# chenxy99/Scanpaths

Hardware: AMD Instinct MI355X
Metric: images/sec/GPU (AiR train step, bs=32, 320x512) at 1/2/4/8 MI355X (higher is better)
Workload: dtype f32; 1 GPU; AiR supervised train step (fwd+loss+bwd+clip+Adam), resnet50, T=16, 320x512, per-GPU batch 32; global_batch=32, parallelism=dp1

## Files before the change

scanpaths_amd/csrc/bn_pool.hip:

```cpp
#include "common.h"
#include <algorithm>

namespace {

__device__ __forceinline__ int64_t sp_cdiv_dev(int64_t a, int64_t b) { return (a + b - 1) / b; }

constexpr int CB = 64;
constexpr int RL = 16;
constexpr int MAX_G = 256;

inline int pick_G_wide(int64_t M, int C) {
    const int64_t colblocks = sp_cdiv(C, 256);
    int64_t g = sp_cdiv(1024, colblocks);
    g = std::min<int64_t>(g, sp_cdiv(M, 4 * 8));
    g = std::min<int64_t>(g, 1024);
    return (int)std::max<int64_t>(g, 1);
}

inline int pick_G(int64_t M, int C) {
    const int64_t colblocks = sp_cdiv(C, CB);
    int64_t g = sp_cdiv(2048, colblocks);
    g = std::min<int64_t>(g, sp_cdiv(M, RL * 8));
    g = std::min<int64_t>(g, MAX_G);
    return (int)std::max<int64_t>(g, 1);
// ... 631 lines not shown
__global__ __launch_bounds__(256) void maxpool_fwd_kernel(const float* x, int N, int H, int W, int C, float* y, int Ho,
                                                          int Wo, unsigned char* amx) {
    const int C4 = C / 4;
    const int64_t total = (int64_t)N * Ho * Wo * C4;
    for (int64_t i = (int64_t)blockIdx.x * blockDim.x + threadIdx.x; i < total; i += (int64_t)gridDim.x * blockDim.x) {
        const int c4 = (int)(i % C4);
        int64_t r = i / C4;
        const int xo = (int)(r % Wo); r /= Wo;
        const int yo = (int)(r % Ho);
        const int n = (int)(r / Ho);
        float4 m = make_float4(-INFINITY, -INFINITY, -INFINITY, -INFINITY);
        uchar4 am = make_uchar4(0, 0, 0, 0);
        for (int ky = 0; ky < 3; ++ky) {
            const int iy = yo * 2 + ky;
            if (iy >= H) break;
            for (int kx = 0; kx < 3; ++kx) {
                const int ix = xo * 2 + kx;
                if (ix >= W) break;
                const float4 a = *reinterpret_cast<const float4*>(x + (((int64_t)n * H + iy) * W + ix) * C + c4 * 4);
                const unsigned char q = (unsigned char)(ky * 3 + kx);
                if (a.x > m.x) { m.x = a.x; am.x = q; }
                if (a.y > m.y) { m.y = a.y; am.y = q; }
                if (a.z > m.z) { m.z = a.z; am.z = q; }
                if (a.w > m.w) { m.w = a.w; am.w = q; }
            }
        }
        reinterpret_cast<float4*>(y)[i] = m;
        if (amx) reinterpret_cast<uchar4*>(amx)[i] = am;
    }
}

__global__ __launch_bounds__(256) void maxpool_bwd_idx_kernel(const float* dy, const unsigned char* amx, int N, int H, int W,
                                                              int C, float* dx, int Ho, int Wo) {
    const int C4 = C / 4;
    const int64_t total = (int64_t)N * H * W * C4;
    for (int64_t i = (int64_t)blockIdx.x * blockDim.x + threadIdx.x; i < total; i += (int64_t)gridDim.x * blockDim.x) {
        const int c4 = (int)(i % C4);
        int64_t r = i / C4;
        const int ix = (int)(r % W); r /= W;
        const int iy = (int)(r % H);
        const int n = (int)(r / H);
        float4 g = make_float4(0.f, 0.f, 0.f, 0.f);
        const int oy_lo = max(0, (iy - 1) / 2), oy_hi = min(Ho - 1, iy / 2);
        const int ox_lo = max(0, (ix - 1) / 2), ox_hi = min(Wo - 1, ix / 2);
        for (int oy = oy_lo; oy <= oy_hi; ++oy) {
            if (iy - 2 * oy > 2) continue;
            for (int ox = ox_lo; ox <= ox_hi; ++ox) {
                if (ix - 2 * ox > 2) continue;
                const int64_t o = (((int64_t)n * Ho + oy) * Wo + ox) * C4 + c4;
                const uchar4 a = reinterpret_cast<const uchar4*>(amx)[o];
                const unsigned char mine = (unsigned char)((iy - 2 * oy) * 3 + (ix - 2 * ox));
                if (a.x == mine || a.y == mine || a.z == mine || a.w == mine) {
                    const float4 d = reinterpret_cast<const float4*>(dy)[o];
                    g.x += a.x == mine ? d.x : 0.f;
                    g.y += a.y == mine ? d.y : 0.f;
                    g.z += a.z == mine ? d.z : 0.f;
                    g.w += a.w == mine ? d.w : 0.f;
                }
            }
        }
        reinterpret_cast<float4*>(dx)[i] = g;
    }
}

__global__ __launch_bounds__(256) void nchw_to_nhwc_pad_kernel(const float* x, int N, int C, int H, int W, int Cp, float* y) {
    const int64_t total = (int64_t)N * H * W * Cp;
    for (int64_t i = (int64_t)blockIdx.x * blockDim.x + threadIdx.x; i < total; i += (int64_t)gridDim.x * blockDim.x) {
        const int c = (int)(i % Cp);
        int64_t r = i / Cp;
        const int w = (int)(r % W); r /= W;
        const int hh = (int)(r % H);
        const int n = (int)(r / H);
        y[i] = c < C ? x[(((int64_t)n * C + c) * H + hh) * W + w] : 0.f;
    }
}
__global__ __launch_bounds__(256) void pad_lastdim_kernel(const float* x, int64_t rows, int Cin, int Cout, float* y) {
    const int64_t total = rows * Cout;
    for (int64_t i = (int64_t)blockIdx.x * blockDim.x + threadIdx.x; i < total; i += (int64_t)gridDim.x * blockDim.x) {
        const int c = (int)(i % Cout);
        const int64_t r = i / Cout;
        y[i] = c < Cin ? x[r * Cin + c] : 0.f;
    }
}
__global__ __launch_bounds__(256) void add_kernel(const float* a, const float* b, float* o, int64_t n4) {
    for (int64_t i = (int64_t)blockIdx.x * blockDim.x + threadIdx.x; i < n4; i += (int64_t)gridDim.x * blockDim.x) {
        const float4 u = reinterpret_cast<const float4*>(a)[i], v = reinterpret_cast<const float4*>(b)[i];
        reinterpret_cast<float4*>(o)[i] = make_float4(u.x + v.x, u.y + v.y, u.z + v.z, u.w + v.w);
    }
}
struct SumList {
    const float* p[32];
    int n;
    const int* row_last;
    int step[32];
// ... 262 lines not shown
extern "C" int sp_rowsum(const float* x, int64_t M, int C, float scale, float* out, void* stream) {
    if (!x || !out) return SP_ENULL;
    if (C % 4) return SP_EINVAL;
    const int blocks = (int)std::max<int64_t>(1, std::min<int64_t>(sp_cdiv(M, 4), 4096));
    hipLaunchKernelGGL(rowsum_kernel, dim3(blocks), dim3(256), 0, (hipStream_t)stream, x, M, C, scale, out);
    SP_LAUNCH_CHECK();
    return SP_OK;
}

extern "C" int sp_rowsum_bwd(const float* dout, int64_t M, int C, float scale, float* dx, void* stream) {
    if (!dout || !dx) return SP_ENULL;
    if (C % 4) return SP_EINVAL;
    const int64_t n4 = M * C / 4;
    hipLaunchKernelGGL(rowsum_bwd_kernel, dim3(ew_blocks(n4)), dim3(256), 0, (hipStream_t)stream, dout, n4, C, scale, dx);
    SP_LAUNCH_CHECK();
    return SP_OK;
}

extern "C" int sp_maxpool3s2_fwd(const float* x, int N, int H, int W, int C, float* y, unsigned char* argmax, int Ho, int Wo,
                                 void* stream) {
    if (!x || !y) return SP_ENULL;
    if (C % 4) return SP_EINVAL;
    const int64_t total = (int64_t)N * Ho * Wo * (C / 4);
    hipLaunchKernelGGL(maxpool_fwd_kernel, dim3(ew_blocks(total)), dim3(256), 0, (hipStream_t)stream, x, N, H, W, C, y, Ho, Wo,
                       argmax);
    SP_LAUNCH_CHECK();
    return SP_OK;
}

extern "C" int sp_maxpool3s2_bwd(const float* dy, const unsigned char* argmax, int N, int H, int W, int C, float* dx, int Ho,
                                 int Wo, void* stream) {
    if (!dy || !argmax || !dx) return SP_ENULL;
    if (C % 4) return SP_EINVAL;
    const int64_t total = (int64_t)N * H * W * (C / 4);
    hipLaunchKernelGGL(maxpool_bwd_idx_kernel, dim3(ew_blocks(total) * 4), dim3(256), 0, (hipStream_t)stream, dy, argmax, N, H, W,
                       C, dx, Ho, Wo);
    SP_LAUNCH_CHECK();
    return SP_OK;
}

extern "C" int sp_nchw_to_nhwc_pad(const float* x, int N, int C, int H, int W, int Cp, float* y, void* stream) {
    if (!x || !y) return SP_ENULL;
    if (Cp < C) return SP_EINVAL;
    const int64_t total = (int64_t)N * H * W * Cp;
    hipLaunchKernelGGL(nchw_to_nhwc_pad_kernel, dim3(ew_blocks(total)), dim3(256), 0, (hipStream_t)stream, x, N, C, H, W, Cp, y);
    SP_LAUNCH_CHECK();
    return SP_OK;
}

extern "C" int sp_pad_lastdim(const float* x, int64_t rows, int Cin, int Cout, float* y, void* stream) {
    if (!x || !y) return SP_ENULL;
    const int64_t total = rows * Cout;
    hipLaunchKernelGGL(pad_lastdim_kernel, dim3(ew_blocks(total)), dim3(256), 0, (hipStream_t)stream, x, rows, Cin, Cout, y);
    SP_LAUNCH_CHECK();
    return SP_OK;
}

extern "C" int sp_add(const float* a, const float* b, float* out, int64_t n, void* stream) {
    if (!a || !b || !out) return SP_ENULL;
    const int64_t n4 = n / 4;
    if (n4 > 0) {
        hipLaunchKernelGGL(add_kernel, dim3(ew_blocks(n4)), dim3(256), 0, (hipStream_t)stream, a, b, out, n4);
        SP_LAUNCH_CHECK();
    }
    if (n4 * 4 < n) {
        hipLaunchKernelGGL(add_tail_kernel, dim3(1), dim3(256), 0, (hipStream_t)stream, a, b, out, n4 * 4, n);
        SP_LAUNCH_CHECK();
// ... 57 lines not shown
```

scanpaths_amd/csrc/decoder.hip:

```cpp
#include "common.h"
#include <algorithm>

namespace {

inline int ew_blocks(int64_t n) { return (int)std::max<int64_t>(1, std::min<int64_t>(sp_cdiv(n, 256), 2048)); }

__device__ __forceinline__ float sigmoidf_(float x) { return sp_sigmoid(x); }

__global__ __launch_bounds__(256) void lstm_fwd_kernel(const float* xg, const float* hg, const float* c_prev,
                                                       int64_t rows, int C, float* gates, float* c_out, float* h_out) {
    const int C4 = C / 4;
    const int64_t total = rows * C4;
    for (int64_t idx = (int64_t)blockIdx.x * blockDim.x + threadIdx.x; idx < total; idx += (int64_t)gridDim.x * blockDim.x) {
        const int64_t r = idx / C4;
        const int c = (int)(idx - r * C4) * 4;
        const float* px = xg + r * 4 * C + c;
        float4 pi = *reinterpret_cast<const float4*>(px);
        float4 pf = *reinterpret_cast<const float4*>(px + C);
        float4 po = *reinterpret_cast<const float4*>(px + 2 * C);
        float4 pg = *reinterpret_cast<const float4*>(px + 3 * C);
        if (hg) {
            const float* ph = hg + r * 4 * C + c;
            const float4 a = *reinterpret_cast<const float4*>(ph), b = *reinterpret_cast<const float4*>(ph + C);
            const float4 d = *reinterpret_cast<const float4*>(ph + 2 * C), e = *reinterpret_cast<const float4*>(ph + 3 * C);
            pi.x += a.x; pi.y += a.y; pi.z += a.z; pi.w += a.w;
            pf.x += b.x; pf.y += b.y; pf.z += b.z; pf.w += b.w;
            po.x += d.x; po.y += d.y; po.z += d.z; po.w += d.w;
            pg.x += e.x; pg.y += e.y; pg.z += e.z; pg.w += e.w;
        }
        float4 cp = make_float4(0.f, 0.f, 0.f, 0.f);
        if (c_prev) cp = *reinterpret_cast<const float4*>(c_prev + r * C + c);
        float4 gi, gf, go, gg, cn, hn;
#define CELL(k)                                   \
        gi.k = sigmoidf_(pi.k);                   \
        gf.k = sigmoidf_(pf.k);                   \
        go.k = sigmoidf_(po.k);                   \
        gg.k = sp_tanh(pg.k);                       \
        cn.k = gf.k * cp.k + gi.k * gg.k;         \
        hn.k = go.k * cn.k;
        CELL(x) CELL(y) CELL(z) CELL(w)
#undef CELL
        float* pgt = gates + r * 4 * C + c;
        *reinterpret_cast<float4*>(pgt) = gi;
        *reinterpret_cast<float4*>(pgt + C) = gf;
        *reinterpret_cast<float4*>(pgt + 2 * C) = go;
        *reinterpret_cast<float4*>(pgt + 3 * C) = gg;
        *reinterpret_cast<float4*>(c_out + r * C + c) = cn;
        *reinterpret_cast<float4*>(h_out + r * C + c) = hn;
    }
}

constexpr int SP_PCH = 160;
__global__ __launch_bounds__(256) void sempool_fwd_kernel(const float* __restrict__ a, const float* __restrict__ vf, int S, int B,
                                                          int P, int C, float* __restrict__ partial) {
    __shared__ f32x4 red[2][128];
    const int ch = blockIdx.x, b = blockIdx.y, nch = gridDim.x;
    const int c4 = threadIdx.x & 127, pl = threadIdx.x >> 7, C4 = C / 4;
    const int p0 = ch * SP_PCH, p1 = min(P, p0 + SP_PCH);
    f32x4 acc0 = {0.f, 0.f, 0.f, 0.f}, acc1 = {0.f, 0.f, 0.f, 0.f};
    if (c4 < C4)
        for (int p = p0 + pl; p < p1; p += 2) {
            const f32x4 v = *reinterpret_cast<const f32x4*>(vf + ((int64_t)b * P + p) * C + c4 * 4);
            acc0 += a[((int64_t)0 * B + b) * P + p] * v;
            if (S > 1) acc1 += a[((int64_t)1 * B + b) * P + p] * v;
        }
    if (pl == 1) { red[0][c4] = acc0; red[1][c4] = acc1; }
    __syncthreads();
    if (pl == 0 && c4 < C4) {
        acc0 += red[0][c4];
        acc1 += red[1][c4];
        f32x4* dst = reinterpret_cast<f32x4*>(partial + (((int64_t)ch * B + b) * S) * C) + c4;
        dst[0] = acc0;
        if (S > 1) dst[C4] = acc1;
    }
    (void)nch;
}
__global__ __launch_bounds__(256) void sempool_finish_kernel(const float* __restrict__ partial, int nch, int64_t n, float alpha,
                                                             float* __restrict__ out, int S, int C, int64_t osb, int64_t oss) {
    for (int64_t i = (int64_t)blockIdx.x * 256 + threadIdx.x; i < n; i += (int64_t)gridDim.x * 256) {
        float s = 0.f;
        for (int k = 0; k < nch; ++k) s += partial[(int64_t)k * n + i];
        const int c = (int)(i % C);
        const int64_t bs = i / C;
        out[(bs / S) * osb + (bs % S) * oss + c] = fmaxf(alpha * s, 0.f);
    }
}
__global__ __launch_bounds__(256) void sempool_bwd_kernel(const float* __restrict__ dz, const float* __restrict__ out,
                                                          const float* __restrict__ a, const float* __restrict__ vf, int S,
                                                          int B, int P, int C, float alpha, float* __restrict__ da,
                                                          float* __restrict__ dvf, const int* __restrict__ row_last, int row_step,
                                                          int64_t zsb, int64_t zss) {
    const int lane = threadIdx.x & 63;
    const int64_t wave = ((int64_t)blockIdx.x * 256 + threadIdx.x) >> 6, nwaves = ((int64_t)gridDim.x * 256) >> 6;
    const int nq = C / 4;
    for (int64_t bp = wave; bp < (int64_t)B * P; bp += nwaves) {
        const int b = (int)(bp / P), p = (int)(bp % P);
        if (row_last && row_last[b] < row_step) {
            for (int q = lane; q < nq; q += 64) *reinterpret_cast<f32x4*>(dvf + bp * C + q * 4) = f32x4{0.f, 0.f, 0.f, 0.f};
// ... 279 lines not shown
        const int x = (int)(q % W); q /= W;
        const int y = (int)(q % H);
        const int r = (int)(q / H);
        float v = 0.f;
        if (k < 9 * S) {
            const int s = k / 9, tap = k - 9 * s;
            const int yy = y + tap / 3 - 1, xx = x + tap % 3 - 1;
            if ((unsigned)yy < (unsigned)H && (unsigned)xx < (unsigned)W) v = maps[(((int64_t)s * R + r) * H + yy) * W + xx];
        }
        col[i] = v;
    }
}
__global__ __launch_bounds__(256) void col2im1_multi_kernel(const float* __restrict__ dcol, int S, int R, int H, int W, int ldk, float* __restrict__ dmaps) {
    const int64_t total = (int64_t)S * R * H * W;
    for (int64_t i = (int64_t)blockIdx.x * blockDim.x + threadIdx.x; i < total; i += (int64_t)gridDim.x * blockDim.x) {
        int64_t q = i;
        const int x = (int)(q % W); q /= W;
        const int y = (int)(q % H); q /= H;
        const int r = (int)(q % R);
        const int s = (int)(q / R);
        float acc = 0.f;
#pragma unroll
        for (int tap = 0; tap < 9; ++tap) {
            const int y0 = y - (tap / 3 - 1), x0 = x - (tap % 3 - 1);
            if ((unsigned)y0 < (unsigned)H && (unsigned)x0 < (unsigned)W)
                acc += dcol[(((int64_t)r * H + y0) * W + x0) * ldk + 9 * s + tap];
        }
        dmaps[i] = acc;
    }
}

constexpr int MAXT = 40;

__global__ __launch_bounds__(256) void listatt_fwd_kernel(const float* L, const float* u, int T, int R, int D, float* mem,
                                                          float* alpha) {
    __shared__ float sh16[16];
    __shared__ float sc[MAXT];
    const int r = blockIdx.x;
    for (int t0 = 0; t0 < T; t0 += 4) {
        float s[4] = {0.f, 0.f, 0.f, 0.f};
        for (int d = threadIdx.x; d < D; d += 256) {
            const float ud = u[d];
#pragma unroll
            for (int k = 0; k < 4; ++k)
                if (t0 + k < T) s[k] += L[((int64_t)(t0 + k) * R + r) * D + d] * ud;
        }
        block_sum4_256(s, sh16);
        if (threadIdx.x == 0) {
#pragma unroll
            for (int k = 0; k < 4; ++k)
                if (t0 + k < T) sc[t0 + k] = s[k];
        }
    }
    __syncthreads();
    float mx = -INFINITY;
    for (int t = 0; t < T; ++t) mx = fmaxf(mx, sc[t]);
    float den = 0.f;
    for (int t = 0; t < T; ++t) den += expf(sc[t] - mx);
    const float inv = 1.f / den;
    if (threadIdx.x < T) alpha[(int64_t)threadIdx.x * R + r] = expf(sc[threadIdx.x] - mx) * inv;
    for (int d = threadIdx.x; d < D; d += 256) {
        float acc = 0.f;
        for (int t = 0; t < T; ++t) acc += expf(sc[t] - mx) * inv * L[((int64_t)t * R + r) * D + d];
        mem[(int64_t)r * D + d] = acc;
    }
}

__global__ __launch_bounds__(256) void listatt_bwd_kernel(const float* dmem, const float* L, const float* u,
                                                          const float* alpha, int T, int R, int D, float* dL,
                                                          float* du_partial) {
    __shared__ float sh16[16];
    __shared__ float gs[MAXT];
    const int r = blockIdx.x;
    const float* dm = dmem + (int64_t)r * D;
    for (int t0 = 0; t0 < T; t0 += 4) {
        float s[4] = {0.f, 0.f, 0.f, 0.f};
        for (int d = threadIdx.x; d < D; d += 256) {
            const float dmd = dm[d];
#pragma unroll
            for (int k = 0; k < 4; ++k)
                if (t0 + k < T) s[k] += L[((int64_t)(t0 + k) * R + r) * D + d] * dmd;
        }
        block_sum4_256(s, sh16);
        if (threadIdx.x == 0) {
#pragma unroll
            for (int k = 0; k < 4; ++k)
                if (t0 + k < T) gs[t0 + k] = s[k];
        }
    }
    __syncthreads();
    float mean = 0.f;
    for (int t = 0; t < T; ++t) mean += alpha[(int64_t)t * R + r] * gs[t];
    for (int d = threadIdx.x; d < D; d += 256) {
        const float dmd = dm[d], ud = u[d];
        float du = 0.f;
        for (int t = 0; t < T; ++t) {
// ... 310 lines not shown
                                     const unsigned* dc_amax, float c_bound, float cprev_bound, void* planes,
                                     float* dpre_scale, const int* row_last, int row_step, int rows_per_sample, void* stream) {
    if (!gates || !c_out || (!dpre && !planes) || !dc_prev) return SP_ENULL;
    if (C % 4) return SP_EINVAL;
    if (planes && (!dpre_scale || C % 256 || ((uintptr_t)planes & 15) || (dh && !dh_amax) || (dc && !dc_amax))) return SP_EINVAL;
    if (row_last && (rows_per_sample < 1 || rows % rows_per_sample)) return SP_EINVAL;
    SP_RESET_AMAX(dpre_amax, stream);
    SP_RESET_AMAX(dcp_amax, stream);
    hipLaunchKernelGGL(lstm_bwd_kernel, dim3(ew_blocks(rows * C / 4)), dim3(256), 0, (hipStream_t)stream, dh, dc, gates,
                       c_prev, c_out, rows, C, dpre, dc_prev, dpre_amax, dcp_amax, dh_amax, dc_amax, c_bound, cprev_bound,
                       (uint16_t*)planes, dpre_scale, row_last, row_step, row_last ? rows_per_sample : 1);
    SP_LAUNCH_CHECK();
    return SP_OK;
}

extern "C" int sp_im2col3x3_1ch(const float* maps, int S, int R, int H, int W, int ldk, float* col, void* stream) {
    if (!maps || !col) return SP_ENULL;
    if (S < 1 || 9 * S > ldk) return SP_EINVAL;
    hipLaunchKernelGGL(im2col1_multi_kernel, dim3(ew_blocks((int64_t)R * H * W * ldk)), dim3(256), 0, (hipStream_t)stream, maps, S, R, H, W, ldk, col);
    SP_LAUNCH_CHECK();
    return SP_OK;
}
extern "C" int sp_col2im3x3_1ch(const float* dcol, int S, int R, int H, int W, int ldk, float* dmaps, void* stream) {
    if (!dcol || !dmaps) return SP_ENULL;
    if (S < 1 || 9 * S > ldk) return SP_EINVAL;
    hipLaunchKernelGGL(col2im1_multi_kernel, dim3(ew_blocks((int64_t)S * R * H * W)), dim3(256), 0, (hipStream_t)stream, dcol, S, R, H, W, ldk, dmaps);
    SP_LAUNCH_CHECK();
    return SP_OK;
}

extern "C" int sp_listatt_fwd(const float* L, const float* u, int T, int R, int D, float* mem, float* alpha, void* stream) {
    if (!L || !u || !mem || !alpha) return SP_ENULL;
    if (T < 1 || T > MAXT) return SP_EINVAL;
    hipLaunchKernelGGL(listatt_fwd_kernel, dim3(R), dim3(256), 0, (hipStream_t)stream, L, u, T, R, D, mem, alpha);
    SP_LAUNCH_CHECK();
    return SP_OK;
}

extern "C" int sp_listatt_bwd(const float* dmem, const float* L, const float* u, const float* alpha, int T, int R, int D,
                              float* dL, float* du_partial, void* stream) {
    if (!dmem || !L || !u || !alpha || !dL || !du_partial) return SP_ENULL;
    if (T < 1 || T > MAXT) return SP_EINVAL;
    hipLaunchKernelGGL(listatt_bwd_kernel, dim3(R), dim3(256), 0, (hipStream_t)stream, dmem, L, u, alpha, T, R, D, dL,
                       du_partial);
    SP_LAUNCH_CHECK();
    return SP_OK;
}

extern "C" int sp_mulrelu_fwd(const float* a, const float* b, int64_t n, int64_t nb, float* out, void* stream) {
    if (!a || !b || !out) return SP_ENULL;
    hipLaunchKernelGGL(mulrelu_fwd_kernel, dim3(ew_blocks(n)), dim3(256), 0, (hipStream_t)stream, a, b, n, nb, out);
    SP_LAUNCH_CHECK();
    return SP_OK;
}

extern "C" int sp_mulrelu_bwd(const float* dout, const float* a, const float* b, const float* out, int64_t n, int64_t nb,
                              float* da, float* db_partial, void* stream) {
    if (!dout || !a || !b || !out || !da || !db_partial) return SP_ENULL;
    hipLaunchKernelGGL(mulrelu_bwd_kernel, dim3(ew_blocks(n)), dim3(256), 0, (hipStream_t)stream, dout, a, b, out, n, nb, da,
                       db_partial);
    SP_LAUNCH_CHECK();
    return SP_OK;
}

extern "C" int sp_select_rows(const float* a, const float* b, const unsigned char* sel, int64_t rows, int64_t len, float* out,
                              void* stream) {
    if (!a || !b || !sel || !out) return SP_ENULL;
// ... 57 lines not shown
```

scanpaths_amd/csrc/head_direct.hip:

```cpp
#include "common.h"

namespace {

constexpr int NTAP = 49, NV = 121, MAXSITE = 32, MAXCLS = 8;

struct AxisCls {
    int n;
    int ncls;
    int len;
    unsigned char mask[MAXCLS];
    unsigned char cls[MAXSITE];
};

static bool make_axis(int len, AxisCls& a) {
    a.n = sp_drt_sites(len);
    a.ncls = 0;
    a.len = len;
    if (a.n < 1 || a.n > MAXSITE) return false;
    for (int s = 0; s < a.n; ++s) {
        unsigned m = 0;
        for (int k = 0; k < 7; ++k) {
            const int pos = 5 * s - 2 + k;
            if (pos >= 0 && pos < len) m |= 1u << k;
        }
// ... 36 lines not shown
        float s = 0.f;
        for (int ky = 0; ky < 7; ++ky)
            for (int kx = 0; kx < 7; ++kx)
                if (((my >> ky) & 1u) && ((mx >> kx) & 1u)) s += cb[(int64_t)hd * HC + 2 + ky * 7 + kx];
        cbsum[hd * ncls + cls] = s;
    }
}

__global__ __launch_bounds__(128) void compose11_bwd_kernel(const float* __restrict__ dW11, const float* __restrict__ dcbsum,
                                                            int HC, int C4, int ncls, AxisCls ay, AxisCls ax,
                                                            float* __restrict__ dG, float* __restrict__ dcb) {
    const int u = blockIdx.x, tap = blockIdx.y, hd = blockIdx.z;
    const int ky = tap / 7, kx = tap % 7, uy = u / 5, ux = u % 5;
    const int v = (ky + uy) * 11 + kx + ux;
    const f32x4* S4 = reinterpret_cast<const f32x4*>(dW11);
    f32x4* O4 = reinterpret_cast<f32x4*>(dG);
    const int64_t row = (int64_t)hd * HC + 2 + tap;
    for (int c4 = threadIdx.x; c4 < C4; c4 += blockDim.x) {
        f32x4 acc = {0.f, 0.f, 0.f, 0.f};
        for (int cls = 0; cls < ncls; ++cls) {
            if (!((ay.mask[cls / ax.ncls] >> ky) & 1u) || !((ax.mask[cls % ax.ncls] >> kx) & 1u)) continue;
            acc += S4[(((int64_t)hd * ncls + cls) * NV + v) * C4 + c4];
        }
        O4[(row * 25 + u) * C4 + c4] = acc;
    }
    if (u == 0 && threadIdx.x == 0) {
        double s = 0.0;
        for (int cls = 0; cls < ncls; ++cls)
            if (((ay.mask[cls / ax.ncls] >> ky) & 1u) && ((ax.mask[cls % ax.ncls] >> kx) & 1u)) s += (double)dcbsum[hd * ncls + cls];
        dcb[row] = (float)s;
    }
}

__global__ __launch_bounds__(256) void sal_gather_fwd_kernel(const float* __restrict__ T, int B, int Hm, int Wm, int ldt,
                                                             int nsel, const int* __restrict__ hmap, float* __restrict__ Z2) {
    const int P = Hm * Wm, J = nsel * 2;
    const int64_t n = (int64_t)B * P * J;
    for (int64_t i = (int64_t)blockIdx.x * 256 + threadIdx.x; i < n; i += (int64_t)gridDim.x * 256) {
        const int j = (int)(i % J);
        const int64_t bp = i / J;
        const int p = (int)(bp % P), b = (int)(bp / P);
        const int py = p / Wm, px = p % Wm;
        const int col0 = (hmap[b * nsel + (j >> 1)] * 2 + (j & 1)) * 25;
        const float* t = T + (int64_t)b * P * ldt + col0;
        float acc = 0.f;
        for (int uy = 0; uy < 5; ++uy) {
            const int qy = py + uy - 2;
            if ((unsigned)qy >= (unsigned)Hm) continue;
            for (int ux = 0; ux < 5; ++ux) {
                const int qx = px + ux - 2;
                if ((unsigned)qx < (unsigned)Wm) acc += t[(int64_t)(qy * Wm + qx) * ldt + uy * 5 + ux];
            }
        }
        Z2[i] = acc;
    }
}

__global__ __launch_bounds__(256) void sal_gather_bwd_kernel(const float* __restrict__ dZ2, int B, int Hm, int Wm, int ldt,
                                                             int nsel, int nsrc, const int* __restrict__ hmap,
                                                             float* __restrict__ dT, const int* __restrict__ row_last, int row_step) {
    const int P = Hm * Wm, J = nsel * 2;
    const int64_t n = (int64_t)B * P * ldt;
    for (int64_t i = (int64_t)blockIdx.x * 256 + threadIdx.x; i < n; i += (int64_t)gridDim.x * 256) {
        const int col = (int)(i % ldt);
        const int64_t bq = i / ldt;
        const int q = (int)(bq % P), b = (int)(bq / P);
        float v = 0.f;
        if (col < nsrc * 50 && !(row_last && row_last[b] < row_step)) {
            const int src = col / 50, o = (col % 50) / 25, u = col % 25;
            const int py = q / Wm - (u / 5 - 2), px = q % Wm - (u % 5 - 2);
            if ((unsigned)py < (unsigned)Hm && (unsigned)px < (unsigned)Wm)
                for (int s = 0; s < nsel; ++s)
                    if (hmap[b * nsel + s] == src) v += dZ2[((int64_t)b * P + py * Wm + px) * J + s * 2 + o];
        }
        dT[i] = v;
    }
}

constexpr int DRT_GB = 4;
__device__ __forceinline__ float drt_dot4(const f32x4& a, const f32x4& w, float acc) {
    return __builtin_fmaf(a[3], w[3], __builtin_fmaf(a[2], w[2], __builtin_fmaf(a[1], w[1], __builtin_fmaf(a[0], w[0], acc))));
}
__global__ __launch_bounds__(256) void drt_fwd_kernel(const float* __restrict__ h, const float* __restrict__ W11,
                                                      const float* __restrict__ cbsum, const int* __restrict__ hmap, int B,
                                                      int C4, int nsel, int ncls, AxisCls ay, AxisCls ax,
                                                      float* __restrict__ Dpre) {
    __shared__ float sh4[4];
    int s = blockIdx.x, gy = blockIdx.y;
    if (ay.n == 8 && ((gridDim.x * gridDim.y) & 7u) == 0) {
        const unsigned bid = blockIdx.y * gridDim.x + blockIdx.x, q = bid >> 3;
        s = (int)(bid & 7u) * ax.n + (int)(q % (unsigned)ax.n);
        gy = (int)(q / (unsigned)ax.n);
    }
    const int b0 = gy * DRT_GB, i0 = blockIdx.z * 2;
    const int nb = min(DRT_GB, B - b0);
    const bool two = i0 + 1 < nsel;
    const int Hm = ay.len, Wm = ax.len, S = ay.n * ax.n;
    const int sy = s / ax.n, sx = s % ax.n;
    const int cls = ay.cls[sy] * ax.ncls + ax.cls[sx];
    const int oy = 5 * sy - 4, ox = 5 * sx - 4;
    int src0[DRT_GB], src1[DRT_GB];
    bool same = true;
#pragma unroll
    for (int j = 0; j < DRT_GB; ++j) {
        const int b = min(b0 + j, B - 1);
        src0[j] = hmap[b * nsel + i0];
        src1[j] = two ? hmap[b * nsel + i0 + 1] : src0[j];
        same = same && src0[j] == src0[0] && src1[j] == src1[0];
    }
    const int64_t wstride = (int64_t)ncls * NV * C4;
    const f32x4* W4c = reinterpret_cast<const f32x4*>(W11) + (int64_t)cls * NV * C4;
    const f32x4* H4 = reinterpret_cast<const f32x4*>(h);
    const int64_t hb = (int64_t)Hm * Wm * C4;
    float acc0[DRT_GB], acc1[DRT_GB];
#pragma unroll
    for (int j = 0; j < DRT_GB; ++j) acc0[j] = acc1[j] = 0.f;
    const int vy0 = max(0, -oy), vy1 = min(10, Hm - 1 - oy), vx0 = max(0, -ox), vx1 = min(10, Wm - 1 - ox);
    const int nvx = vx1 - vx0 + 1, cnt = max(0, vy1 - vy0 + 1) * max(0, nvx);
#pragma unroll 4
    for (int it = threadIdx.x; it < cnt * C4; it += 256) {
        const int k = it / C4, c4 = it - k * C4;
        const int ky = k / nvx, vy = vy0 + ky, vx = vx0 + (k - ky * nvx);
        const int idx = (vy * 11 + vx) * C4 + c4;
        const int64_t ho = (int64_t)((oy + vy) * Wm + ox + vx) * C4 + c4;
        f32x4 a[DRT_GB];
#pragma unroll
        for (int j = 0; j < DRT_GB; ++j) a[j] = H4[(int64_t)min(b0 + j, B - 1) * hb + ho];
        if (same) {
            const f32x4 w = W4c[src0[0] * wstride + idx];
#pragma unroll
            for (int j = 0; j < DRT_GB; ++j) acc0[j] = drt_dot4(a[j], w, acc0[j]);
            if (two) {
                const f32x4 u = W4c[src1[0] * wstride + idx];
#pragma unroll
                for (int j = 0; j < DRT_GB; ++j) acc1[j] = drt_dot4(a[j], u, acc1[j]);
            }
        } else {
#pragma unroll
            for (int j = 0; j < DRT_GB; ++j) {
                const f32x4 w = W4c[src0[j] * wstride + idx];
                acc0[j] = drt_dot4(a[j], w, acc0[j]);
                if (two) {
                    const f32x4 u = W4c[src1[j] * wstride + idx];
                    acc1[j] = drt_dot4(a[j], u, acc1[j]);
                }
            }
        }
    }
#pragma unroll
    for (int j = 0; j < DRT_GB; ++j) {
        if (j >= nb) break;
        const float r0 = block_sum_256(acc0[j], sh4);
        const float r1 = two ? block_sum_256(acc1[j], sh4) : 0.f;
        if (threadIdx.x == 0) {
            Dpre[((int64_t)i0 * B + b0 + j) * S + s] = r0 + cbsum[src0[j] * ncls + cls];
            if (two) Dpre[((int64_t)(i0 + 1) * B + b0 + j) * S + s] = r1 + cbsum[src1[j] * ncls + cls];
        }
    }
}

__device__ __forceinline__ bool drt_row_dead(const int* __restrict__ row_last, int row_step, int rowB, int b) {
    return row_last != nullptr && row_last[b % rowB] < row_step + b / rowB;
}

__global__ __launch_bounds__(256, 6) void drt_bwd_data_kernel(const float* __restrict__ dD, const float* __restrict__ W11,
                                                           const int* __restrict__ hmap, int B, int C4, int nsel, int ncls,
                                                           AxisCls ay, AxisCls ax, int accumulate, float* __restrict__ dh,
                                                           const int* __restrict__ live, const int* __restrict__ row_last, int row_step,
                                                           int rowB) {
    const int Hm = ay.len, Wm = ax.len, P = Hm * Wm, S = ay.n * ax.n;
    const f32x4* W4 = reinterpret_cast<const f32x4*>(W11);
    f32x4* O4 = reinterpret_cast<f32x4*>(dh);
    const int NG = (B + DRT_GB - 1) / DRT_GB;
    const int64_t n = (int64_t)NG * P * C4;
    for (int64_t t = (int64_t)blockIdx.x * 256 + threadIdx.x; t < n; t += (int64_t)gridDim.x * 256) {
        const int c4 = (int)(t % C4);
        const int64_t gq = t / C4;
        const int q = (int)(gq % P), b0 = (int)(gq / P) * DRT_GB;
        const int nb = min(DRT_GB, B - b0);
        const int qy = q / Wm, qx = q % Wm;
        f32x4 acc[DRT_GB];
#pragma unroll
        for (int j = 0; j < DRT_GB; ++j) acc[j] = f32x4{0.f, 0.f, 0.f, 0.f};
        unsigned on = 0;
        for (int i = 0; i < nsel && i < 8; ++i)
#pragma unroll
            for (int j = 0; j < DRT_GB; ++j)
                if (j < nb && !drt_row_dead(row_last, row_step, rowB, b0 + j) && (!live || live[(int64_t)i * B + b0 + j])) on |= 1u << (i * DRT_GB + j);
        const bool flagged = (live != nullptr || row_last != nullptr) && nsel <= 8;
// ... 139 lines not shown
    return ay.ncls * ax.ncls;
}

extern "C" int sp_head_compose11_fwd(const float* G, const float* cb, int nheads, int HC, int C, int Hm, int Wm, float* W11,
                                     float* cbsum, void* stream) {
    if (!G || !cb || !W11 || !cbsum) return SP_ENULL;
    AxisCls ay, ax;
    if (HC < 2 + NTAP || C % 4 || nheads < 1 || !make_axis(Hm, ay) || !make_axis(Wm, ax)) return SP_EINVAL;
    hipLaunchKernelGGL(compose11_fwd_kernel, dim3(NV, ay.ncls * ax.ncls, nheads), dim3(128), 0, (hipStream_t)stream, G, cb, HC,
                       C / 4, ay, ax, W11, cbsum);
    SP_LAUNCH_CHECK();
    return SP_OK;
}

extern "C" int sp_head_compose11_bwd(const float* dW11, const float* dcbsum, int nheads, int HC, int C, int Hm, int Wm,
                                     float* dG, float* dcb, void* stream) {
    if (!dW11 || !dcbsum || !dG || !dcb) return SP_ENULL;
    AxisCls ay, ax;
    if (HC < 2 + NTAP || C % 4 || nheads < 1 || !make_axis(Hm, ay) || !make_axis(Wm, ax)) return SP_EINVAL;
    hipError_t e = hipMemsetAsync(dG, 0, (size_t)nheads * HC * 25 * C * sizeof(float), (hipStream_t)stream);
    if (e != hipSuccess) return (int)e;
    e = hipMemsetAsync(dcb, 0, (size_t)nheads * HC * sizeof(float), (hipStream_t)stream);
    if (e != hipSuccess) return (int)e;
    hipLaunchKernelGGL(compose11_bwd_kernel, dim3(25, NTAP, nheads), dim3(128), 0, (hipStream_t)stream, dW11, dcbsum, HC, C / 4,
                       ay.ncls * ax.ncls, ay, ax, dG, dcb);
    SP_LAUNCH_CHECK();
    return SP_OK;
}

extern "C" int sp_sal_gather_fwd(const float* T, int B, int Hm, int Wm, int ldt, int nsel, const int* hmap, float* Z2,
                                 void* stream) {
    if (!T || !hmap || !Z2) return SP_ENULL;
    if (B < 1 || nsel < 1 || ldt < 50) return SP_EINVAL;
    hipLaunchKernelGGL(sal_gather_fwd_kernel, dim3(ew_grid((int64_t)B * Hm * Wm * nsel * 2)), dim3(256), 0, (hipStream_t)stream,
                       T, B, Hm, Wm, ldt, nsel, hmap, Z2);
    SP_LAUNCH_CHECK();
    return SP_OK;
}

extern "C" int sp_sal_gather_bwd(const float* dZ2, int B, int Hm, int Wm, int ldt, int nsel, int nsrc, const int* hmap,
                                 float* dT, const int* row_last, int row_step, void* stream) {
    if (!dZ2 || !hmap || !dT) return SP_ENULL;
    if (B < 1 || nsel < 1 || nsrc < 1 || ldt < nsrc * 50) return SP_EINVAL;
    hipLaunchKernelGGL(sal_gather_bwd_kernel, dim3(ew_grid((int64_t)B * Hm * Wm * ldt)), dim3(256), 0, (hipStream_t)stream, dZ2,
                       B, Hm, Wm, ldt, nsel, nsrc, hmap, dT, row_last, row_step);
    SP_LAUNCH_CHECK();
    return SP_OK;
}

extern "C" int sp_drt_direct_fwd(const float* h, const float* W11, const float* cbsum, const int* hmap, int B, int Hm, int Wm,
                                 int C, int nsel, float* Dpre, void* stream) {
    if (!h || !W11 || !cbsum || !hmap || !Dpre) return SP_ENULL;
    AxisCls ay, ax;
    if (C % 4 || B < 1 || nsel < 1 || !make_axis(Hm, ay) || !make_axis(Wm, ax)) return SP_EINVAL;
    hipLaunchKernelGGL(drt_fwd_kernel, dim3(ay.n * ax.n, (B + DRT_GB - 1) / DRT_GB, (nsel + 1) / 2), dim3(256), 0, (hipStream_t)stream, h, W11, cbsum, hmap, B,
                       C / 4, nsel, ay.ncls * ax.ncls, ay, ax, Dpre);
    SP_LAUNCH_CHECK();
    return SP_OK;
}

extern "C" int sp_drt_direct_bwd_data(const float* dDpre, const float* W11, const int* hmap, int B, int Hm, int Wm, int C,
                                      int nsel, int accumulate, float* dh, const int* live, const int* row_last, int row_step, int rowB,
                                      void* stream) {
    if (!dDpre || !W11 || !hmap || !dh) return SP_ENULL;
    AxisCls ay, ax;
    if (C % 4 || B < 1 || nsel < 1 || !make_axis(Hm, ay) || !make_axis(Wm, ax)) return SP_EINVAL;
    if (row_last && (rowB < 1 || B % rowB)) return SP_EINVAL;
    hipLaunchKernelGGL(drt_bwd_data_kernel, dim3(ew_grid((int64_t)((B + DRT_GB - 1) / DRT_GB) * Hm * Wm * (C / 4))), dim3(256), 0, (hipStream_t)stream,
                       dDpre, W11, hmap, B, C / 4, nsel, ay.ncls * ax.ncls, ay, ax, accumulate, dh, live, row_last, row_step, row_last ? rowB : B);
    SP_LAUNCH_CHECK();
    return SP_OK;
}

extern "C" int64_t sp_drt_direct_bwd_weight_workspace(int B, int Hm, int Wm, int C, int nsel) {
    AxisCls ay, ax;
    if (!make_axis(Hm, ay) || !make_axis(Wm, ax)) return -1;
    return (int64_t)B * nsel * ay.ncls * ax.ncls * NV * C * (int64_t)sizeof(float);
}

extern "C" int sp_drt_direct_bwd_weight(const float* dDpre, const float* h, const int* hmap, int B, int Hm, int Wm, int C,
                                        int nsel, int nheads, void* workspace, float* dW11, float* dcbsum, const int* live,
                                        const int* row_last, int row_step, int rowB, void* stream) {
    if (!dDpre || !h || !hmap || !workspace || !dW11 || !dcbsum) return SP_ENULL;
    AxisCls ay, ax;
    if (C % 4 || B < 1 || nsel < 1 || nheads < 1 || !make_axis(Hm, ay) || !make_axis(Wm, ax)) return SP_EINVAL;
    if (row_last && (rowB < 1 || B % rowB)) return SP_EINVAL;
    if (!row_last) rowB = B;
    const int ncls = ay.ncls * ax.ncls;
// ... 13 lines not shown
```

Measured before the change: 144.9 images/s.

## Rework maxpool bwd, sempool, listatt, sal_gather and drt kernels for reuse

Several unrelated kernels are restructured. Maxpool backward now has each thread cover a 2x2 input patch, loading the shared output windows once. Sempool forward unrolls its loop by eight with explicit FMAs. Listatt forward uses 1024-thread blocks with 16 scores per pass and caches softmax weights, sal_gather stages a halo tile in shared memory, and drt forward handles seven horizontal sites per block with software-prefetched loads. Together these aim to cut redundant global loads and launch overhead, at the cost of higher register and shared-memory pressure.

```diff
diff --git a/scanpaths_amd/csrc/bn_pool.hip b/scanpaths_amd/csrc/bn_pool.hip
--- a/scanpaths_amd/csrc/bn_pool.hip
+++ b/scanpaths_amd/csrc/bn_pool.hip
@@ -687,34 +687,48 @@
 
 __global__ __launch_bounds__(256) void maxpool_bwd_idx_kernel(const float* dy, const unsigned char* amx, int N, int H, int W,
                                                               int C, float* dx, int Ho, int Wo) {
-    const int C4 = C / 4;
-    const int64_t total = (int64_t)N * H * W * C4;
+    const int C4 = C / 4, Ha = (H + 1) / 2, Wa = (W + 1) / 2;
+    const int64_t total = (int64_t)N * Ha * Wa * C4;
     for (int64_t i = (int64_t)blockIdx.x * blockDim.x + threadIdx.x; i < total; i += (int64_t)gridDim.x * blockDim.x) {
         const int c4 = (int)(i % C4);
         int64_t r = i / C4;
-        const int ix = (int)(r % W); r /= W;
-        const int iy = (int)(r % H);
-        const int n = (int)(r / H);
-        float4 g = make_float4(0.f, 0.f, 0.f, 0.f);
-        const int oy_lo = max(0, (iy - 1) / 2), oy_hi = min(Ho - 1, iy / 2);
-        const int ox_lo = max(0, (ix - 1) / 2), ox_hi = min(Wo - 1, ix / 2);
-        for (int oy = oy_lo; oy <= oy_hi; ++oy) {
-            if (iy - 2 * oy > 2) continue;
-            for (int ox = ox_lo; ox <= ox_hi; ++ox) {
-                if (ix - 2 * ox > 2) continue;
-                const int64_t o = (((int64_t)n * Ho + oy) * Wo + ox) * C4 + c4;
-                const uchar4 a = reinterpret_cast<const uchar4*>(amx)[o];
-                const unsigned char mine = (unsigned char)((iy - 2 * oy) * 3 + (ix - 2 * ox));
-                if (a.x == mine || a.y == mine || a.z == mine || a.w == mine) {
-                    const float4 d = reinterpret_cast<const float4*>(dy)[o];
-                    g.x += a.x == mine ? d.x : 0.f;
-                    g.y += a.y == mine ? d.y : 0.f;
-                    g.z += a.z == mine ? d.z : 0.f;
-                    g.w += a.w == mine ? d.w : 0.f;
-                }
-            }
-        }
-        reinterpret_cast<float4*>(dx)[i] = g;
+        const int b = (int)(r % Wa); r /= Wa;
+        const int a = (int)(r % Ha);
+        const int n = (int)(r / Ha);
+        uchar4 am[2][2];
+        float4 d[2][2];
+#pragma unroll
+        for (int wy = 0; wy < 2; ++wy)
+#pragma unroll
+            for (int wx = 0; wx < 2; ++wx) {
+                const int oy = a - 1 + wy, ox = b - 1 + wx;
+                const bool ok = oy >= 0 && oy < Ho && ox >= 0 && ox < Wo;
+                const int64_t o = (((int64_t)n * Ho + min(max(oy, 0), Ho - 1)) * Wo + min(max(ox, 0), Wo - 1)) * C4 + c4;
+                const uchar4 q = reinterpret_cast<const uchar4*>(amx)[o];
+                am[wy][wx] = ok ? q : make_uchar4(255, 255, 255, 255);
+                d[wy][wx] = reinterpret_cast<const float4*>(dy)[o];
+            }
+#pragma unroll
+        for (int py = 0; py < 2; ++py)
+#pragma unroll
+            for (int px = 0; px < 2; ++px) {
+                const int iy = 2 * a + py, ix = 2 * b + px;
+                if (iy >= H || ix >= W) continue;
+                float4 g = make_float4(0.f, 0.f, 0.f, 0.f);
+#pragma unroll
+                for (int wy = py; wy < 2; ++wy)
+#pragma unroll
+                    for (int wx = px; wx < 2; ++wx) {
+                        const unsigned char mine = (unsigned char)((py + 2 - 2 * wy) * 3 + (px + 2 - 2 * wx));
+                        const uchar4 q = am[wy][wx];
+                        const float4 v = d[wy][wx];
+                        g.x += q.x == mine ? v.x : 0.f;
+                        g.y += q.y == mine ? v.y : 0.f;
+                        g.z += q.z == mine ? v.z : 0.f;
+                        g.w += q.w == mine ? v.w : 0.f;
+                    }
+                reinterpret_cast<float4*>(dx)[(((int64_t)n * H + iy) * W + ix) * C4 + c4] = g;
+            }
     }
 }
 
@@ -1043,7 +1057,7 @@
                                  int Wo, void* stream) {
     if (!dy || !argmax || !dx) return SP_ENULL;
     if (C % 4) return SP_EINVAL;
-    const int64_t total = (int64_t)N * H * W * (C / 4);
+    const int64_t total = (int64_t)N * ((H + 1) / 2) * ((W + 1) / 2) * (C / 4);
     hipLaunchKernelGGL(maxpool_bwd_idx_kernel, dim3(ew_blocks(total) * 4), dim3(256), 0, (hipStream_t)stream, dy, argmax, N, H, W,
                        C, dx, Ho, Wo);
     SP_LAUNCH_CHECK();
diff --git a/scanpaths_amd/csrc/decoder.hip b/scanpaths_amd/csrc/decoder.hip
--- a/scanpaths_amd/csrc/decoder.hip
+++ b/scanpaths_amd/csrc/decoder.hip
@@ -51,6 +51,11 @@
 }
 
 constexpr int SP_PCH = 160;
+constexpr int SP_UNR = 8;
+__device__ __forceinline__ f32x4 sp_fma4(float x, const f32x4& v, const f32x4& acc) {
+    return f32x4{__builtin_fmaf(x, v[0], acc[0]), __builtin_fmaf(x, v[1], acc[1]), __builtin_fmaf(x, v[2], acc[2]),
+                 __builtin_fmaf(x, v[3], acc[3])};
+}
 __global__ __launch_bounds__(256) void sempool_fwd_kernel(const float* __restrict__ a, const float* __restrict__ vf, int S, int B,
                                                           int P, int C, float* __restrict__ partial) {
     __shared__ f32x4 red[2][128];
@@ -58,12 +63,32 @@
     const int c4 = threadIdx.x & 127, pl = threadIdx.x >> 7, C4 = C / 4;
     const int p0 = ch * SP_PCH, p1 = min(P, p0 + SP_PCH);
     f32x4 acc0 = {0.f, 0.f, 0.f, 0.f}, acc1 = {0.f, 0.f, 0.f, 0.f};
-    if (c4 < C4)
-        for (int p = p0 + pl; p < p1; p += 2) {
-            const f32x4 v = *reinterpret_cast<const f32x4*>(vf + ((int64_t)b * P + p) * C + c4 * 4);
-            acc0 += a[((int64_t)0 * B + b) * P + p] * v;
-            if (S > 1) acc1 += a[((int64_t)1 * B + b) * P + p] * v;
-        }
+    if (c4 < C4) {
+        const float* a0p = a + (int64_t)b * P;
+        const float* a1p = a + ((int64_t)B + b) * P;
+        const float* vp = vf + (int64_t)b * P * C + c4 * 4;
+        int p = p0 + pl;
+        for (; p + 2 * (SP_UNR - 1) < p1; p += 2 * SP_UNR) {
+            f32x4 v[SP_UNR];
+            float x0[SP_UNR], x1[SP_UNR];
+#pragma unroll
+            for (int k = 0; k < SP_UNR; ++k) {
+                v[k] = *reinterpret_cast<const f32x4*>(vp + (int64_t)(p + 2 * k) * C);
+                x0[k] = a0p[p + 2 * k];
+                x1[k] = S > 1 ? a1p[p + 2 * k] : 0.f;
+            }
+#pragma unroll
+            for (int k = 0; k < SP_UNR; ++k) {
+                acc0 = sp_fma4(x0[k], v[k], acc0);
+                if (S > 1) acc1 = sp_fma4(x1[k], v[k], acc1);
+            }
+        }
+        for (; p < p1; p += 2) {
+            const f32x4 v = *reinterpret_cast<const f32x4*>(vp + (int64_t)p * C);
+            acc0 = sp_fma4(a0p[p], v, acc0);
+            if (S > 1) acc1 = sp_fma4(a1p[p], v, acc1);
+        }
+    }
     if (pl == 1) { red[0][c4] = acc0; red[1][c4] = acc1; }
     __syncthreads();
     if (pl == 0 && c4 < C4) {
@@ -409,24 +434,50 @@
 
 constexpr int MAXT = 40;
 
-__global__ __launch_bounds__(256) void listatt_fwd_kernel(const float* L, const float* u, int T, int R, int D, float* mem,
-                                                          float* alpha) {
-    __shared__ float sh16[16];
+constexpr int LA_NT = 1024, LA_NW = LA_NT / 64, LA_RT = 16;
+
+template <int K>
+__device__ __forceinline__ void listatt_scores(const float* L, const float* u, int t0, int T, int R, int D, int r, float (&s)[LA_RT]) {
+    const float* row[K];
+#pragma unroll
+    for (int k = 0; k < K; ++k) row[k] = L + ((int64_t)min(t0 + k, T - 1) * R + r) * D;
+    for (int d = threadIdx.x; d < D; d += LA_NT) {
+        const float ud = u[d];
+        float x[K];
+#pragma unroll
+        for (int k = 0; k < K; ++k) x[k] = row[k][d];
+#pragma unroll
+        for (int k = 0; k < K; ++k) s[k] += x[k] * ud;
+    }
+#pragma unroll
+    for (int k = 0; k < K; ++k) s[k] = wave_sum(s[k]);
+}
+
+__global__ __launch_bounds__(LA_NT) void listatt_fwd_kernel(const float* L, const float* u, int T, int R, int D, float* mem,
+                                                            float* alpha) {
+    __shared__ float part[LA_NW][LA_RT];
     __shared__ float sc[MAXT];
-    const int r = blockIdx.x;
-    for (int t0 = 0; t0 < T; t0 += 4) {
-        float s[4] = {0.f, 0.f, 0.f, 0.f};
-        for (int d = threadIdx.x; d < D; d += 256) {
-            const float ud = u[d];
-#pragma unroll
-            for (int k = 0; k < 4; ++k)
-                if (t0 + k < T) s[k] += L[((int64_t)(t0 + k) * R + r) * D + d] * ud;
-        }
-        block_sum4_256(s, sh16);
-        if (threadIdx.x == 0) {
-#pragma unroll
-            for (int k = 0; k < 4; ++k)
-                if (t0 + k < T) sc[t0 + k] = s[k];
+    __shared__ float wt[MAXT];
+    const int r = blockIdx.x, tid = threadIdx.x;
+    for (int t0 = 0; t0 < T; t0 += LA_RT) {
+        const int nt = min(LA_RT, T - t0);
+        float s[LA_RT];
+#pragma unroll
+        for (int k = 0; k < LA_RT; ++k) s[k] = 0.f;
+        if (nt <= 4) listatt_scores<4>(L, u, t0, T, R, D, r, s);
+        else if (nt <= 8) listatt_scores<8>(L, u, t0, T, R, D, r, s);
+        else listatt_scores<LA_RT>(L, u, t0, T, R, D, r, s);
+        __syncthreads();
+        if ((tid & 63) == 0) {
+#pragma unroll
+            for (int k = 0; k < LA_RT; ++k) part[tid >> 6][k] = s[k];
+        }
+        __syncthreads();
+        if (tid < nt) {
+            float v = 0.f;
+#pragma unroll
+            for (int w = 0; w < LA_NW; ++w) v += part[w][tid];
+            sc[t0 + tid] = v;
         }
     }
     __syncthreads();
@@ -435,10 +486,22 @@
     float den = 0.f;
     for (int t = 0; t < T; ++t) den += expf(sc[t] - mx);
     const float inv = 1.f / den;
-    if (threadIdx.x < T) alpha[(int64_t)threadIdx.x * R + r] = expf(sc[threadIdx.x] - mx) * inv;
-    for (int d = threadIdx.x; d < D; d += 256) {
+    if (tid < T) {
+        const float a = expf(sc[tid] - mx) * inv;
+        wt[tid] = a;
+        alpha[(int64_t)tid * R + r] = a;
+    }
+    __syncthreads();
+    for (int d = tid; d < D; d += LA_NT) {
         float acc = 0.f;
-        for (int t = 0; t < T; ++t) acc += expf(sc[t] - mx) * inv * L[((int64_t)t * R + r) * D + d];
+        for (int t0 = 0; t0 < T; t0 += 8) {
+            float x[8];
+#pragma unroll
+            for (int k = 0; k < 8; ++k) x[k] = L[((int64_t)min(t0 + k, T - 1) * R + r) * D + d];
+#pragma unroll
+            for (int k = 0; k < 8; ++k)
+                if (t0 + k < T) acc += wt[t0 + k] * x[k];
+        }
         mem[(int64_t)r * D + d] = acc;
     }
 }
@@ -815,7 +878,7 @@
 extern "C" int sp_listatt_fwd(const float* L, const float* u, int T, int R, int D, float* mem, float* alpha, void* stream) {
     if (!L || !u || !mem || !alpha) return SP_ENULL;
     if (T < 1 || T > MAXT) return SP_EINVAL;
-    hipLaunchKernelGGL(listatt_fwd_kernel, dim3(R), dim3(256), 0, (hipStream_t)stream, L, u, T, R, D, mem, alpha);
+    hipLaunchKernelGGL(listatt_fwd_kernel, dim3(R), dim3(LA_NT), 0, (hipStream_t)stream, L, u, T, R, D, mem, alpha);
     SP_LAUNCH_CHECK();
     return SP_OK;
 }
diff --git a/scanpaths_amd/csrc/head_direct.hip b/scanpaths_amd/csrc/head_direct.hip
--- a/scanpaths_amd/csrc/head_direct.hip
+++ b/scanpaths_amd/csrc/head_direct.hip
@@ -92,27 +92,50 @@
     }
 }
 
+constexpr int SG_TR = 8, SG_TC = 32, SG_SC = SG_TC + 4, SG_NPIX = (SG_TR + 4) * SG_SC, SG_LD = 8;
 __global__ __launch_bounds__(256) void sal_gather_fwd_kernel(const float* __restrict__ T, int B, int Hm, int Wm, int ldt,
                                                              int nsel, const int* __restrict__ hmap, float* __restrict__ Z2) {
+    __shared__ float tile[SG_NPIX * 25];
     const int P = Hm * Wm, J = nsel * 2;
-    const int64_t n = (int64_t)B * P * J;
-    for (int64_t i = (int64_t)blockIdx.x * 256 + threadIdx.x; i < n; i += (int64_t)gridDim.x * 256) {
-        const int j = (int)(i % J);
-        const int64_t bp = i / J;
-        const int p = (int)(bp % P), b = (int)(bp / P);
-        const int py = p / Wm, px = p % Wm;
+    const int ntx = (Wm + SG_TC - 1) / SG_TC;
+    const int tx = blockIdx.x % ntx, ty = blockIdx.x / ntx, j = blockIdx.y;
+    const int y0 = ty * SG_TR - 2, x0 = tx * SG_TC - 2;
+    const int oy = threadIdx.x / SG_TC, ox = threadIdx.x % SG_TC;
+    const int py = ty * SG_TR + oy, px = tx * SG_TC + ox;
+    for (int b = blockIdx.z; b < B; b += gridDim.z) {
         const int col0 = (hmap[b * nsel + (j >> 1)] * 2 + (j & 1)) * 25;
         const float* t = T + (int64_t)b * P * ldt + col0;
+        for (int e0 = 0; e0 < SG_NPIX * 25; e0 += 256 * SG_LD) {
+            float v[SG_LD];
+#pragma unroll
+            for (int k = 0; k < SG_LD; ++k) {
+                const int e = min(e0 + k * 256 + (int)threadIdx.x, SG_NPIX * 25 - 1);
+                const int pix = e / 25, tap = e - pix * 25;
+                const int ry = pix / SG_SC, qy = y0 + ry, qx = x0 + pix - ry * SG_SC;
+                const bool in = (unsigned)qy < (unsigned)Hm && (unsigned)qx < (unsigned)Wm;
+                const float x = t[(int64_t)(min(max(qy, 0), Hm - 1) * Wm + min(max(qx, 0), Wm - 1)) * ldt + tap];
+                v[k] = in ? x : 0.f;
+            }
+#pragma unroll
+            for (int k = 0; k < SG_LD; ++k) {
+                const int e = e0 + k * 256 + (int)threadIdx.x;
+                if (e < SG_NPIX * 25) tile[e] = v[k];
+            }
+        }
+        __syncthreads();
         float acc = 0.f;
+#pragma unroll
         for (int uy = 0; uy < 5; ++uy) {
             const int qy = py + uy - 2;
             if ((unsigned)qy >= (unsigned)Hm) continue;
+#pragma unroll
             for (int ux = 0; ux < 5; ++ux) {
                 const int qx = px + ux - 2;
-                if ((unsigned)qx < (unsigned)Wm) acc += t[(int64_t)(qy * Wm + qx) * ldt + uy * 5 + ux];
-            }
-        }
-        Z2[i] = acc;
+                if ((unsigned)qx < (unsigned)Wm) acc += tile[((oy + uy) * SG_SC + ox + ux) * 25 + uy * 5 + ux];
+            }
+        }
+        if (py < Hm && px < Wm) Z2[((int64_t)b * P + py * Wm + px) * J + j] = acc;
+        __syncthreads();
     }
 }
 
@@ -137,7 +160,7 @@
     }
 }
 
-constexpr int DRT_GB = 4;
+constexpr int DRT_GB = 4, DRT_NS = 7;
 __device__ __forceinline__ float drt_dot4(const f32x4& a, const f32x4& w, float acc) {
     return __builtin_fmaf(a[3], w[3], __builtin_fmaf(a[2], w[2], __builtin_fmaf(a[1], w[1], __builtin_fmaf(a[0], w[0], acc))));
 }
@@ -145,20 +168,15 @@
                                                       const float* __restrict__ cbsum, const int* __restrict__ hmap, int B,
                                                       int C4, int nsel, int ncls, AxisCls ay, AxisCls ax,
                                                       float* __restrict__ Dpre) {
-    __shared__ float sh4[4];
-    int s = blockIdx.x, gy = blockIdx.y;
-    if (ay.n == 8 && ((gridDim.x * gridDim.y) & 7u) == 0) {
-        const unsigned bid = blockIdx.y * gridDim.x + blockIdx.x, q = bid >> 3;
-        s = (int)(bid & 7u) * ax.n + (int)(q % (unsigned)ax.n);
-        gy = (int)(q / (unsigned)ax.n);
-    }
-    const int b0 = gy * DRT_GB, i0 = blockIdx.z * 2;
+    __shared__ float sh16[16];
+    const int nch = (ax.n + DRT_NS - 1) / DRT_NS;
+    const int sy = blockIdx.x / nch, sx0 = (blockIdx.x % nch) * DRT_NS;
+    const int nsx = min(DRT_NS, ax.n - sx0);
+    const int b0 = blockIdx.y * DRT_GB, i0 = blockIdx.z * 2;
     const int nb = min(DRT_GB, B - b0);
     const bool two = i0 + 1 < nsel;
     const int Hm = ay.len, Wm = ax.len, S = ay.n * ax.n;
-    const int sy = s / ax.n, sx = s % ax.n;
-    const int cls = ay.cls[sy] * ax.ncls + ax.cls[sx];
-    const int oy = 5 * sy - 4, ox = 5 * sx - 4;
+    const int oy = 5 * sy - 4, ox = 5 * sx0 - 4;
     int src0[DRT_GB], src1[DRT_GB];
     bool same = true;
 #pragma unroll
@@ -168,53 +186,89 @@
         src1[j] = two ? hmap[b * nsel + i0 + 1] : src0[j];
         same = same && src0[j] == src0[0] && src1[j] == src1[0];
     }
+    int cls[DRT_NS];
+#pragma unroll
+    for (int s = 0; s < DRT_NS; ++s) cls[s] = ay.cls[sy] * ax.ncls + ax.cls[min(sx0 + s, ax.n - 1)];
     const int64_t wstride = (int64_t)ncls * NV * C4;
-    const f32x4* W4c = reinterpret_cast<const f32x4*>(W11) + (int64_t)cls * NV * C4;
+    const f32x4* W4 = reinterpret_cast<const f32x4*>(W11);
     const f32x4* H4 = reinterpret_cast<const f32x4*>(h);
     const int64_t hb = (int64_t)Hm * Wm * C4;
-    float acc0[DRT_GB], acc1[DRT_GB];
-#pragma unroll
-    for (int j = 0; j < DRT_GB; ++j) acc0[j] = acc1[j] = 0.f;
-    const int vy0 = max(0, -oy), vy1 = min(10, Hm - 1 - oy), vx0 = max(0, -ox), vx1 = min(10, Wm - 1 - ox);
-    const int nvx = vx1 - vx0 + 1, cnt = max(0, vy1 - vy0 + 1) * max(0, nvx);
-#pragma unroll 4
-    for (int it = threadIdx.x; it < cnt * C4; it += 256) {
-        const int k = it / C4, c4 = it - k * C4;
-        const int ky = k / nvx, vy = vy0 + ky, vx = vx0 + (k - ky * nvx);
-        const int idx = (vy * 11 + vx) * C4 + c4;
-        const int64_t ho = (int64_t)((oy + vy) * Wm + ox + vx) * C4 + c4;
-        f32x4 a[DRT_GB];
-#pragma unroll
-        for (int j = 0; j < DRT_GB; ++j) a[j] = H4[(int64_t)min(b0 + j, B - 1) * hb + ho];
-        if (same) {
-            const f32x4 w = W4c[src0[0] * wstride + idx];
-#pragma unroll
-            for (int j = 0; j < DRT_GB; ++j) acc0[j] = drt_dot4(a[j], w, acc0[j]);
-            if (two) {
-                const f32x4 u = W4c[src1[0] * wstride + idx];
-#pragma unroll
-                for (int j = 0; j < DRT_GB; ++j) acc1[j] = drt_dot4(a[j], u, acc1[j]);
-            }
-        } else {
+    float acc0[DRT_NS][DRT_GB], acc1[DRT_NS][DRT_GB];
+#pragma unroll
+    for (int s = 0; s < DRT_NS; ++s)
+#pragma unroll
+        for (int j = 0; j < DRT_GB; ++j) acc0[s][j] = acc1[s][j] = 0.f;
+    const int vy0 = max(0, -oy), vy1 = min(10, Hm - 1 - oy), ux0 = max(0, -ox), ux1 = min(5 * nsx + 5, Wm - 1 - ox);
+    const int nux = max(0, ux1 - ux0 + 1), nvy = max(0, vy1 - vy0 + 1);
+    const int ql = min(C4, 256), npl = 256 / ql;
+    const int pl = threadIdx.x / ql, cq = threadIdx.x - pl * ql;
+    if (pl < npl && nux > 0) {
+        int ky = 0, kx = pl, c4 = cq;
+        while (kx >= nux) { kx -= nux; ++ky; }
+        f32x4 a[DRT_GB], an[DRT_GB];
+        if (ky < nvy) {
+            const int64_t ho = (int64_t)((oy + vy0 + ky) * Wm + ox + ux0 + kx) * C4 + c4;
+#pragma unroll
+            for (int j = 0; j < DRT_GB; ++j) a[j] = H4[(int64_t)min(b0 + j, B - 1) * hb + ho];
+        }
+        while (ky < nvy) {
+            int nky = ky, nkx = kx, nc4 = c4 + 256;
+            if (nc4 >= C4) {
+                nc4 = cq;
+                nkx += npl;
+                while (nkx >= nux) { nkx -= nux; ++nky; }
+            }
+            const bool more = nky < nvy;
+            {
+                const int64_t ho = (int64_t)((oy + vy0 + (more ? nky : ky)) * Wm + ox + ux0 + (more ? nkx : kx)) * C4 + (more ? nc4 : c4);
+#pragma unroll
+                for (int j = 0; j < DRT_GB; ++j) an[j] = H4[(int64_t)min(b0 + j, B - 1) * hb + ho];
+            }
+            const int vy = vy0 + ky, ux = ux0 + kx;
+#pragma unroll
+            for (int s = 0; s < DRT_NS; ++s) {
+                const int vx = ux - 5 * s;
+                if (s >= nsx || vx < 0 || vx > 10) continue;
+                const f32x4* Wc = W4 + ((int64_t)cls[s] * NV + vy * 11 + vx) * C4 + c4;
+                if (same) {
+                    const f32x4 w = Wc[src0[0] * wstride];
+#pragma unroll
+                    for (int j = 0; j < DRT_GB; ++j) acc0[s][j] = drt_dot4(a[j], w, acc0[s][j]);
+                    if (two) {
+                        const f32x4 u = Wc[src1[0] * wstride];
+#pragma unroll
+                        for (int j = 0; j < DRT_GB; ++j) acc1[s][j] = drt_dot4(a[j], u, acc1[s][j]);
+                    }
+                } else {
+#pragma unroll
+                    for (int j = 0; j < DRT_GB; ++j) {
+                        const f32x4 w = Wc[src0[j] * wstride];
+                        acc0[s][j] = drt_dot4(a[j], w, acc0[s][j]);
+                        if (two) {
+                            const f32x4 u = Wc[src1[j] * wstride];
+                            acc1[s][j] = drt_dot4(a[j], u, acc1[s][j]);
+                        }
+                    }
+                }
+            }
+#pragma unroll
+            for (int j = 0; j < DRT_GB; ++j) a[j] = an[j];
+            ky = nky; kx = nkx; c4 = nc4;
+        }
+    }
+#pragma unroll
+    for (int s = 0; s < DRT_NS; ++s) {
+        if (s >= nsx) break;
+        const int site = sy * ax.n + sx0 + s;
+        block_sum4_256(acc0[s], sh16);
+        if (two) block_sum4_256(acc1[s], sh16);
+        if (threadIdx.x == 0) {
 #pragma unroll
             for (int j = 0; j < DRT_GB; ++j) {
-                const f32x4 w = W4c[src0[j] * wstride + idx];
-                acc0[j] = drt_dot4(a[j], w, acc0[j]);
-                if (two) {
-                    const f32x4 u = W4c[src1[j] * wstride + idx];
-                    acc1[j] = drt_dot4(a[j], u, acc1[j]);
-                }
-            }
-        }
-    }
-#pragma unroll
-    for (int j = 0; j < DRT_GB; ++j) {
-        if (j >= nb) break;
-        const float r0 = block_sum_256(acc0[j], sh4);
-        const float r1 = two ? block_sum_256(acc1[j], sh4) : 0.f;
-        if (threadIdx.x == 0) {
-            Dpre[((int64_t)i0 * B + b0 + j) * S + s] = r0 + cbsum[src0[j] * ncls + cls];
-            if (two) Dpre[((int64_t)(i0 + 1) * B + b0 + j) * S + s] = r1 + cbsum[src1[j] * ncls + cls];
+                if (j >= nb) break;
+                Dpre[((int64_t)i0 * B + b0 + j) * S + site] = acc0[s][j] + cbsum[src0[j] * ncls + cls[s]];
+                if (two) Dpre[((int64_t)(i0 + 1) * B + b0 + j) * S + site] = acc1[s][j] + cbsum[src1[j] * ncls + cls[s]];
+            }
         }
     }
 }
@@ -420,7 +474,9 @@
                                  void* stream) {
     if (!T || !hmap || !Z2) return SP_ENULL;
     if (B < 1 || nsel < 1 || ldt < 50) return SP_EINVAL;
-    hipLaunchKernelGGL(sal_gather_fwd_kernel, dim3(ew_grid((int64_t)B * Hm * Wm * nsel * 2)), dim3(256), 0, (hipStream_t)stream,
+    if (Hm < 1 || Wm < 1 || nsel > 32767) return SP_EINVAL;
+    const int tiles = ((Hm + SG_TR - 1) / SG_TR) * ((Wm + SG_TC - 1) / SG_TC);
+    hipLaunchKernelGGL(sal_gather_fwd_kernel, dim3(tiles, nsel * 2, B < 65535 ? B : 65535), dim3(256), 0, (hipStream_t)stream,
                        T, B, Hm, Wm, ldt, nsel, hmap, Z2);
     SP_LAUNCH_CHECK();
     return SP_OK;
@@ -441,7 +497,7 @@
     if (!h || !W11 || !cbsum || !hmap || !Dpre) return SP_ENULL;
     AxisCls ay, ax;
     if (C % 4 || B < 1 || nsel < 1 || !make_axis(Hm, ay) || !make_axis(Wm, ax)) return SP_EINVAL;
-    hipLaunchKernelGGL(drt_fwd_kernel, dim3(ay.n * ax.n, (B + DRT_GB - 1) / DRT_GB, (nsel + 1) / 2), dim3(256), 0, (hipStream_t)stream, h, W11, cbsum, hmap, B,
+    hipLaunchKernelGGL(drt_fwd_kernel, dim3(ay.n * ((ax.n + DRT_NS - 1) / DRT_NS), (B + DRT_GB - 1) / DRT_GB, (nsel + 1) / 2), dim3(256), 0, (hipStream_t)stream, h, W11, cbsum, hmap, B,
                        C / 4, nsel, ay.ncls * ax.ncls, ay, ax, Dpre);
     SP_LAUNCH_CHECK();
     return SP_OK;
```

New measurement: 146.6 images/s, median of 6. 1.01x the previous value.
